# janelia-flyem/flypylib

Hardware: AMD Instinct MI355X
Metric: inference Mvoxels/sec, vgg_like (rf 18, 22^3 coarse -> 88^3 per reference tile), synthetic EM uint8 volume (higher is better)
Workload: dtype f16s; 1 GPU; the 520^3 volume of BASELINE.json's metric (configs[0]'s substack size) per GPU: vgg_like inference, 520x520x520 synthetic uint8 volume, reference tile lattice 102^3 (pitch 88), u8 in / f32 out resident in HBM; tile_in=102, executor=vgg_split_f16, parallelism=z-slab tile sharding x1, no collective, device=AMD Radeon Graphics (gfx950:sramecc+:xnack-)

## Files before the change

flypylib_amd/csrc/vgg_split.hip:

```cpp
#define FPL_F16 1
#include <algorithm>
#include <cmath>

#include "fast_paths.h"
#include "mfma_util.h"
#include "pack_weights.h"
#include <type_traits>
#include "vgg_split_lds.h"
#include "vgg_tiles.h"

namespace {

constexpr int CH = 48;
constexpr int CHP = 24, NPASS = CH / CHP;
constexpr int LO_OFF = CHP * 2;
constexpr int PASS_BYTES = 2 * LO_OFF;
constexpr int VOX = NPASS * PASS_BYTES;
constexpr int KS = (27 * CHP + 31) / 32;
constexpr int KTAB = (KS + 4) / 4 * 4;
constexpr int KTAB_BYTES = 4 * KTAB * 4;
static_assert(CHP % 8 == 0, "a lane's 8 k-slots stay inside one tap");

__host__ __device__ constexpr int64_t chan_off(int ch, int64_t plane) { return (ch / CHP) * plane + (ch % CHP) * 2; }

__device__ __forceinline__ h16x8 pack_relu_split_x(const f32x4 &blk) {
  u32x4 v;
  Pair2 p;
  p = split_pk_relu(blk[0], blk[1]); v[0] = p.hi; v[2] = p.lo;
  p = split_pk_relu(blk[2], blk[3]); v[1] = p.hi; v[3] = p.lo;
  return __builtin_bit_cast(h16x8, v);
}
__device__ __forceinline__ h16x8 pack_relu_split_x(const f32x4 &blk, unsigned &ovf) {
  const h16x8 r = pack_relu_split_x(blk);
  const u32x4 v = __builtin_bit_cast(u32x4, r);
  ovf_note(ovf, pk_max_i16(v[0], v[1]));
  return r;
}

__device__ __forceinline__ f32x4 chain48(const h16x8 (&w)[4], const Frag2 &h01, h16x8 hx, f32x4 acc) {
  acc = mfma16(w[1], h01.hi, acc);
  acc = mfma16(w[0], h01.lo, acc);
  acc = mfma16(w[2], hx, acc);
  acc = mfma16(w[3], hx, acc);
  return mfma16(w[0], h01.hi, acc);
}

__device__ __forceinline__ void store_split12(unsigned char *vox, int64_t plane, int g, const f32x4 (&v)[3],
                                              unsigned &ovf) {
  unsigned hi[6], lo[6];
#pragma unroll
  for (int b = 0; b < 3; ++b) {
    const Pair2 p0 = split_pk(v[b][0], v[b][1], ovf), p1 = split_pk(v[b][2], v[b][3], ovf);
    hi[2 * b] = p0.hi; hi[2 * b + 1] = p1.hi;
    lo[2 * b] = p0.lo; lo[2 * b + 1] = p1.lo;
  }
  unsigned char *d = vox + (g >> 1) * plane + 24 * (g & 1);
  *reinterpret_cast<u32x4_a8 *>(d) = u32x4_a8{hi[0], hi[1], hi[2], hi[3]};
  *reinterpret_cast<u32x2 *>(d + 16) = u32x2{hi[4], hi[5]};
  *reinterpret_cast<u32x4_a8 *>(d + LO_OFF) = u32x4_a8{lo[0], lo[1], lo[2], lo[3]};
  *reinterpret_cast<u32x2 *>(d + LO_OFF + 16) = u32x2{lo[4], lo[5]};
}

constexpr int S_PZ = 4, S_PY = 8, S_PX = 32;
constexpr int S_TZ = 2 * S_PZ + 2, S_TY = 2 * S_PY + 2, S_TX = 2 * S_PX + 2;
constexpr int S_TP = 80;
constexpr int S_TILE = S_TZ * S_TY * S_TP;
constexpr int S_WAVES = 8;
constexpr int S_ROWS = S_TZ * S_TY;
constexpr int S_WROWS = (S_ROWS + S_WAVES - 1) / S_WAVES;
constexpr int S_TASKS = S_PZ * S_PY * 2 / S_WAVES;
constexpr int S_RPT = 3;
static_assert(S_RPT * S_TASKS >= S_WROWS && S_WROWS <= 64, "stem fill schedule");
constexpr int S_SHTAB = 64 * 48;
constexpr int S_SH2 = 4 * 12;
constexpr int S_SMEM = 4 * S_TILE * 2 + 256 * 4 + S_SHTAB * 4 + 2 * S_SH2 * 4;

struct StemSArgs {
  const void *src;
  int64_t SZ, SY, SX;
  int64_t z_hi;
  float mean, sd;
  float c0;
  const float *shtab;
  int64_t p1z0;
  const h16x8 *w1, *w2;
  const float *shift1, *shift2;
  x8::Tensor p1;
  int nbx, nby, nbz;
  unsigned *flag;
  float xlim;
  unsigned char *dump;
};

__device__ __forceinline__ int stem_row_off(int row) {
  return ((row / 3) * S_TY + row % 3) * S_TP;
}

struct StemBlock {
  int px0, py0, pz0;
  int64_t gz0, gy0, gx0;
  unsigned xc;
  bool x_ok;
};

__device__ __forceinline__ StemBlock stem_block(const StemSArgs &a, int q, int lane) {
  StemBlock b;
  const int xb = q % a.nbx, t = q / a.nbx;
  const int yb = t % a.nby, zb = t / a.nby;
  b.px0 = xb * S_PX; b.py0 = yb * S_PY; b.pz0 = zb * S_PZ;
  b.gz0 = 2 * (a.p1z0 + b.pz0); b.gy0 = 2 * (int64_t)b.py0; b.gx0 = 2 * (int64_t)b.px0;
  const int64_t x = b.gx0 + lane;
  b.x_ok = x < a.SX;
  b.xc = (unsigned)(b.x_ok ? x : a.SX - 1);
  return b;
}

__device__ __forceinline__ int stem_row_of(int wrow0, int l) {
  const int r = wrow0 + (l < S_WROWS ? l : S_WROWS - 1);
  return r < S_ROWS ? r : S_ROWS - 1;
}

template <typename SRC>
__device__ __forceinline__ unsigned stem_row_tab(const StemSArgs &a, const StemBlock &b, int wrow0,
                                                 int lane, const SRC *&base) {
  const int row = stem_row_of(wrow0, lane);
  const int64_t z = b.gz0 + row / S_TY, y = b.gy0 + row % S_TY;
  const bool ok = z < a.z_hi && y < a.SY;
  const int64_t zc = z < a.z_hi ? z : a.z_hi - 1, yc = y < a.SY ? y : a.SY - 1;
  const int64_t zb = b.gz0 < a.z_hi ? b.gz0 : a.z_hi - 1, yb = b.gy0 < a.SY ? b.gy0 : a.SY - 1;
  base = (const SRC *)a.src + (zb * a.SY + yb) * a.SX;
  const unsigned rel = (unsigned)(((zc - zb) * a.SY + (yc - yb)) * a.SX);
  return rel | (ok ? 0x80000000u : 0u);
}

template <typename SRC>
struct StemRows {
  SRC v[S_RPT];
  bool ok[S_RPT];
};

template <typename SRC>
__device__ __forceinline__ void stem_load_rows(const SRC *base, unsigned tab, unsigned xc,
                                               int idx0, StemRows<SRC> &r) {
#pragma unroll
  for (int k = 0; k < S_RPT; ++k) {
    const int idx = idx0 + k < S_WROWS ? idx0 + k : S_WROWS - 1;
    const unsigned t = (unsigned)__builtin_amdgcn_readlane((int)tab, idx);
    r.ok[k] = (t >> 31) != 0u;
    r.v[k] = (base + (t & 0x7FFFFFFFu))[xc];
  }
}

template <typename SRC>
__device__ __forceinline__ unsigned stem_norm(const StemSArgs &a, const unsigned *lut, SRC v,
                                              bool ok, unsigned &xmax) {
  unsigned t;
  if (sizeof(SRC) == 1) {
    t = lut[(unsigned)v & 255u];
  } else {
    const float x = ((float)v - a.mean) / a.sd;
    const unsigned ax = __builtin_bit_cast(unsigned, x) & 0x7FFFFFFFu;
    xmax = ax > xmax ? ax : xmax;
    const h16_t h = (h16_t)x;
    t = (unsigned)h16_bits(x) | ((unsigned)h16_bits(x - (float)h) << 16);
  }
  return ok ? t : 0u;
}

struct StemBits { unsigned b[S_RPT]; };

template <typename SRC>
__device__ __forceinline__ void stem_convert_rows(const StemSArgs &a, const StemBlock &b,
                                                  const unsigned *lut, const StemRows<SRC> &r,
                                                  StemBits &o, unsigned &xmax) {
#pragma unroll
  for (int k = 0; k < S_RPT; ++k) o.b[k] = stem_norm<SRC>(a, lut, r.v[k], r.ok[k] && b.x_ok, xmax);
}

template <bool LO>
__device__ __forceinline__ void stem_write_rows(unsigned short *tile, int wrow0, int idx0, int lane,
                                                const StemBits &o) {
#pragma unroll
  for (int k = 0; k < S_RPT; ++k) {
    const int e = stem_row_of(wrow0, idx0 + k) * S_TP + lane;
    tile[e] = (unsigned short)o.b[k];
    if (LO) tile[S_TILE + e] = (unsigned short)(o.b[k] >> 16);
  }
}

template <typename SRC>
struct StemEdge { SRC v[2]; bool ok[2]; };

template <typename SRC>
__device__ __forceinline__ void stem_load_edge(const StemSArgs &a, const StemBlock &b, int wrow0,
                                               int lane, StemEdge<SRC> &e) {
  const int row = stem_row_of(wrow0, lane);
  const int64_t z = b.gz0 + row / S_TY, y = b.gy0 + row % S_TY;
  const bool rok = z < a.z_hi && y < a.SY;
  const int64_t zc = z < a.z_hi ? z : a.z_hi - 1, yc = y < a.SY ? y : a.SY - 1;
  const SRC *rp = (const SRC *)a.src + (zc * a.SY + yc) * a.SX;
#pragma unroll
  for (int j = 0; j < 2; ++j) {
    const int64_t x = b.gx0 + 64 + j;
    e.ok[j] = rok && x < a.SX;
    e.v[j] = rp[x < a.SX ? x : a.SX - 1];
  }
}

template <typename SRC>
__device__ __forceinline__ void stem_store_edge(const StemSArgs &a, unsigned short *tile,
                                                const unsigned *lut, int wrow0, int lane,
                                                const StemEdge<SRC> &e, unsigned &xmax) {
  const int row = stem_row_of(wrow0, lane);
  const unsigned v0 = stem_norm<SRC>(a, lut, e.v[0], e.ok[0], xmax);
  const unsigned v1 = stem_norm<SRC>(a, lut, e.v[1], e.ok[1], xmax);
  *reinterpret_cast<unsigned *>(&tile[row * S_TP + 64]) = (v0 & 0xFFFFu) | (v1 << 16);
  if (sizeof(SRC) != 1)
    *reinterpret_cast<unsigned *>(&tile[S_TILE + row * S_TP + 64]) = (v0 >> 16) | (v1 & 0xFFFF0000u);
}

extern __shared__ __attribute__((aligned(16))) unsigned char smem[];

template <typename SRC>
__global__ __launch_bounds__(64 * S_WAVES, 2) void vggs_stem_pool(StemSArgs a) {
  unsigned short *tiles = reinterpret_cast<unsigned short *>(smem);
  unsigned *lut = reinterpret_cast<unsigned *>(smem + 4 * S_TILE * 2);
  const int tid = threadIdx.x, lane = tid & 63;
  const int wave = __builtin_amdgcn_readfirstlane(tid >> 6);
  const int c = lane & 15, g = lane >> 4;
  const int nblocks = a.nbx * a.nby * a.nbz;
  int q = blockIdx.x;
  if (q >= nblocks) return;
  constexpr bool INT = sizeof(SRC) == 1;
  if (INT && tid < 256) lut[tid] = (unsigned)h16_bits((float)tid - a.c0);
  const unsigned char *shtab = smem + 4 * S_TILE * 2 + 256 * 4;
  if (INT)
    for (int i = tid; i < S_SHTAB; i += 64 * S_WAVES)
      reinterpret_cast<float *>(smem + 4 * S_TILE * 2 + 256 * 4)[i] = a.shtab[i];

  int offP[2][3], offS[2][2];
#pragma unroll
  for (int e = 0; e < 2; ++e) {
#pragma unroll
    for (int i = 0; i < 3; ++i)
      offP[e][i] = 2 * (g < 3 ? stem_row_off(3 * g + i) + (e == 0 ? 0 : 2)
                              : stem_row_off(6 + i) + (e == 0 ? 2 : 0));
#pragma unroll
    for (int h = 0; h < 2; ++h)
      offS[e][h] = 2 * (stem_row_off(2 * (g < 3 ? g : 2) + h) + (e == 0 ? 2 : 1));
  }
  h16x8 w1[2][2][3], w2[4][3];
  float *sh2t = reinterpret_cast<float *>(smem + 4 * S_TILE * 2 + 256 * 4 + S_SHTAB * 4);
  if (tid < S_SH2) {
    const float v = a.shift2[x8::out_channel((tid % 12) / 4, tid / 12, tid % 4)];
    sh2t[tid] = v;
    sh2t[S_SH2 + tid] = -v;
  }
  const f32x4 *sh2g = reinterpret_cast<const f32x4 *>(sh2t + 12 * g);
  const f32x4 *sh2n = reinterpret_cast<const f32x4 *>(sh2t + S_SH2 + 12 * g);
  f32x4 sh1[3];
#pragma unroll
  for (int p = 0; p < 2; ++p)
#pragma unroll
    for (int s = 0; s < 2; ++s)
#pragma unroll
      for (int b = 0; b < 3; ++b) {
        w1[p][s][b] = a.w1[((p * 2 + s) * 3 + b) * 64 + lane];
        w2[2 * p + s][b] = a.w2[((2 * p + s) * 3 + b) * 64 + lane];
      }
#pragma unroll
  for (int b = 0; b < 3; ++b)
#pragma unroll
    for (int r = 0; r < 4; ++r) {
      sh1[b][r] = a.shift1[16 * b + 4 * g + r];
    }
  __syncthreads();

  unsigned ovf = 0u, xmax = 0u;
  const int wrow0 = wave * S_WROWS;
  StemBlock blk = stem_block(a, q, lane);
  {
    const SRC *base0;
    const unsigned tab0 = stem_row_tab<SRC>(a, blk, wrow0, lane, base0);
    for (int i0 = 0; i0 < S_WROWS; i0 += S_RPT) {
      StemRows<SRC> rr;
      StemBits hb;
      stem_load_rows<SRC>(base0, tab0, blk.xc, i0, rr);
      stem_convert_rows<SRC>(a, blk, lut, rr, hb, xmax);
      stem_write_rows<!INT>(tiles, wrow0, i0, lane, hb);
    }
    StemEdge<SRC> ee;
    stem_load_edge<SRC>(a, blk, wrow0, lane, ee);
    stem_store_edge<SRC>(a, tiles, lut, wrow0, lane, ee, xmax);
  }
  __syncthreads();

  const int G = (int)gridDim.x;
  auto clampq = [&](int qq, int qlast) { return qq < nblocks ? qq : qlast; };
  StemRows<SRC> rr;
  StemEdge<SRC> ee;
  StemBits hb;
  {
    const StemBlock n0 = stem_block(a, clampq(q + G, q), lane);
    const SRC *bn;
    const unsigned tn = stem_row_tab<SRC>(a, n0, wrow0, lane, bn);
    stem_load_rows<SRC>(bn, tn, n0.xc, 0, rr);
    stem_load_edge<SRC>(a, n0, wrow0, lane, ee);
    stem_convert_rows<SRC>(a, n0, lut, rr, hb, xmax);
    stem_load_rows<SRC>(bn, tn, n0.xc, S_RPT, rr);
    const f32x4 z3[3] = {{0.f, 0.f, 0.f, 0.f}, {0.f, 0.f, 0.f, 0.f}, {0.f, 0.f, 0.f, 0.f}};
    __builtin_amdgcn_sched_barrier(0);
    x8::store12_sel(a.p1, 0, g, z3, ovf, false, a.dump);
  }
  struct Gin {
    unsigned p[INT ? 1 : 2][3], s0[INT ? 1 : 2], s1[INT ? 1 : 2];
  };
  struct Geo { int base, xrel, yrel, zrel, pzl, pyl, xh; };
  int cur = 0;
  for (;;) {
    const int qn = q + G;
    const bool has_next = qn < nblocks;
    const StemBlock nxt = stem_block(a, has_next ? qn : q, lane);
    const StemBlock nx2 = stem_block(a, clampq(qn + G, has_next ? qn : q), lane);
    const SRC *base_n, *base_2;
    const unsigned tab_n = stem_row_tab<SRC>(a, nxt, wrow0, lane, base_n);
    const unsigned tab_2 = stem_row_tab<SRC>(a, nx2, wrow0, lane, base_2);
    const unsigned char *tb = reinterpret_cast<const unsigned char *>(tiles + cur * 2 * S_TILE);
    unsigned short *tnext = tiles + (cur ^ 1) * 2 * S_TILE;
    auto geo = [&](int ti) {
      Geo t;
      const int task = wave + S_WAVES * ti;
      const int row = task >> 1;
      t.xh = task & 1; t.pzl = row / S_PY; t.pyl = row % S_PY;
      t.base = 2 * (((2 * t.pzl) * S_TY + 2 * t.pyl) * S_TP + 2 * (16 * t.xh + c));
      t.xrel = (int)(blk.gx0 + 2 * (16 * t.xh + c) + 3 - a.SX);
      t.yrel = (int)(blk.gy0 + 2 * t.pyl + 3 - a.SY);
      t.zrel = (int)(blk.gz0 + 2 * t.pzl + 3 - a.z_hi);
      return t;
    };
    const bool interior = INT && blk.gx0 + 2 * S_PX + 2 <= a.SX && blk.gy0 + 2 * S_PY + 2 <= a.SY &&
                          blk.gz0 + 2 * S_PZ + 2 <= a.z_hi;
    auto block_pass = [&](auto edge_t) {
      constexpr bool EDGE = decltype(edge_t)::value;
      f32x4 kin[3];
      if (INT && !EDGE) {
#pragma unroll
        for (int b = 0; b < 3; ++b) kin[b] = *reinterpret_cast<const f32x4 *>(shtab + (4 * g) * 4 + 64 * b);
      }
      auto gather = [&](const Geo &t, int sub, Gin &o) {
        const int sp = sub >> 1, e = sub & 1;
        const int so = 2 * ((((sp >> 1) & 1) * S_TY + (sp & 1)) * S_TP);
#pragma unroll
        for (int part = 0; part < (INT ? 1 : 2); ++part) {
          const unsigned char *tp = tb + part * (S_TILE * 2) + t.base + so;
#pragma unroll
          for (int i = 0; i < 3; ++i) o.p[part][i] = *reinterpret_cast<const unsigned *>(tp + offP[e][i]);
          o.s0[part] = *reinterpret_cast<const unsigned short *>(tp + offS[e][0]);
          o.s1[part] = *reinterpret_cast<const unsigned short *>(tp + offS[e][1]);
        }
      };
      auto gather_init = [&](const Geo &t, int sub, f32x4 (&o)[3]) {
        if (INT && EDGE) {
          const int sp = sub >> 1, e = sub & 1;
          const int pzy = 4 * min(max(t.zrel + (sp >> 1), 0), 3) + min(max(t.yrel + (sp & 1), 0), 3);
          const unsigned char *tp = shtab + ((4 * pzy + min(max(t.xrel + e, 0), 3)) * 48 + 4 * g) * 4;
#pragma unroll
          for (int b = 0; b < 3; ++b) o[b] = *reinterpret_cast<const f32x4 *>(tp + 64 * b);
        }
      };
      auto frag = [&](const Gin &gi, int part) {
        const u32x4 raw = {gi.p[part][0], gi.p[part][1], gi.p[part][2], gi.s0[part] | (gi.s1[part] << 16)};
        return __builtin_bit_cast(h16x8, raw);
      };
      constexpr int NC3 = INT ? 6 : 9;
      auto c3 = [&](int i, int e, const f32x4 (&gin)[3], h16x8 bh, h16x8 bl, f32x4 (&o)[3]) {
        const int b = i % 3, grp = i / 3;
        if (grp == 0) o[b] = mfma16(w1[1][e][b], bh, INT ? (EDGE ? gin[b] : kin[b]) : sh1[b]);
        else if (!INT && grp == 1) o[b] = mfma16(w1[0][e][b], bl, o[b]);
        else o[b] = mfma16(w1[0][e][b], bh, o[b]);
      };
      constexpr int NGB = INT ? 2 : 1, DEPTH = NGB + 1;
      Gin Gd[NGB];
      f32x4 gin[3];
      f32x4 a1n[3];
      f32x4 a2[2][3];
      f32x4 poolf[3];
#pragma unroll
      for (int b = 0; b < 3; ++b) poolf[b] = sh2n[b];
#pragma unroll
      for (int e = 0; e < 2; ++e)
#pragma unroll
        for (int b = 0; b < 3; ++b) a2[e][b] = f32x4{0.f, 0.f, 0.f, 0.f};
      {
        const Geo t0 = geo(0);
        gather(t0, 0, Gd[0]);
        gather_init(t0, 0, gin);
        const h16x8 bh = frag(Gd[0], 0), bl = INT ? bh : frag(Gd[0], INT ? 0 : 1);
#pragma unroll
        for (int i = 0; i < NC3; ++i) c3(i, 0, gin, bh, bl, a1n);
        gather_init(t0, 1, gin);
#pragma unroll
        for (int q = 1; q < DEPTH; ++q) gather(t0, q, Gd[q % NGB]);
      }
#pragma unroll 1
      for (int ti = 0; ti < S_TASKS; ++ti) {
        const bool conv2 = ti + 1 >= S_TASKS, load2 = ti + 2 >= S_TASKS;
        const SRC *lbase = load2 ? base_2 : base_n;
        const unsigned ltab = load2 ? tab_2 : tab_n, lxc = load2 ? nx2.xc : nxt.xc;
        const int lidx = S_RPT * ((ti + 2) & (S_TASKS - 1));
        const Geo tg = geo(ti), tn = geo((ti + 1) & (S_TASKS - 1)), tp = geo((ti + S_TASKS - 1) & (S_TASKS - 1));
#pragma unroll
        for (int sub = 0; sub < 8; ++sub) {
          const int sp = sub >> 1, e = sub & 1, en = e ^ 1;
          f32x4 a1[3];
#pragma unroll
          for (int b = 0; b < 3; ++b) a1[b] = a1n[b];
          const Gin &G = Gd[(sub + 1) % NGB];
          const h16x8 bh = frag(G, 0), bl = INT ? bh : frag(G, INT ? 0 : 1);
          float r[12];
          unsigned hi[6], lo[6];
          auto A = [&](int p) {
            r[2 * p] = relu_f32(a1[p >> 1][2 * (p & 1)]);
            r[2 * p + 1] = relu_f32(a1[p >> 1][2 * (p & 1) + 1]);
            hi[p] = cvt_pk_h16(r[2 * p], r[2 * p + 1]);
          };
          auto B = [&](int p) {
            lo[p] = split_lo_pk(r[2 * p], hi[p], r[2 * p + 1]);
          };
          auto PL = [&](int k) {
#pragma unroll
            for (int j = 2 * k; j < 2 * k + 2; ++j)
              poolf[j >> 2][j & 3] = __builtin_fmaxf(__builtin_fmaxf(poolf[j >> 2][j & 3], a2[0][j >> 2][j & 3]),
                                                     a2[1][j >> 2][j & 3]);
          };
          auto c1 = [&](int i) {
            const int b = i % 3, grp = i / 3;
            const u32x4 h0h = {hi[0], hi[1], hi[2], hi[3]}, h0l = {lo[0], lo[1], lo[2], lo[3]};
            const u32x4 hxv = {hi[4], hi[5], lo[4], lo[5]};
            if (grp == 0) a2[e][b] = mfma16(w2[1][b], __builtin_bit_cast(h16x8, h0h), f32x4{0.f, 0.f, 0.f, 0.f});
            if (grp == 1) a2[e][b] = mfma16(w2[0][b], __builtin_bit_cast(h16x8, h0h), a2[e][b]);
            if (grp == 2) a2[e][b] = mfma16(w2[0][b], __builtin_bit_cast(h16x8, h0l), a2[e][b]);
            if (grp == 3) a2[e][b] = mfma16(w2[2][b], __builtin_bit_cast(h16x8, hxv), a2[e][b]);
            if (grp == 4) a2[e][b] = mfma16(w2[3][b], __builtin_bit_cast(h16x8, hxv), a2[e][b]);
          };
#pragma unroll
          for (int s = 0; s < 15; ++s) {
            if (s < 6) c3(s, en, gin, bh, bl, a1n);
            else c1(s - 6);
            if (s < 6 && e == 0) PL(s);
            if (s < 4) A(s);
            else if (s < 8) B(s - 4);
            else if (s < 10) A(s - 4);
            else if (s < 12) B(s - 6);
            __builtin_amdgcn_sched_barrier(0);
          }
          if (sub + DEPTH < 8) gather(tg, sub + DEPTH, Gd[(sub + DEPTH) % NGB]);
          else gather(tn, sub + DEPTH - 8, Gd[(sub + DEPTH) % NGB]);
          if (sub + 2 < 8) gather_init(tg, sub + 2, gin);
          else gather_init(tn, sub + 2 - 8, gin);
#pragma unroll
          for (int i = 6; i < NC3; ++i) c3(i, en, gin, bh, bl, a1n);
#pragma unroll
          for (int i = 9; i < 15; ++i) c1(i);
          if (sub == 0) {
            const int pz = blk.pz0 + tp.pzl, py = blk.py0 + tp.pyl, px = blk.px0 + 16 * tp.xh + c;
            f32x4 pv[3];
#pragma unroll
            for (int b = 0; b < 3; ++b) pv[b] = poolf[b] + sh2g[b];
            x8::store12_sel(a.p1, a.p1.vox(pz, py, px), g, pv, ovf,
                            ti > 0 && pz < a.p1.Z && py < a.p1.Y && px < a.p1.X, a.dump);
#pragma unroll
            for (int b = 0; b < 3; ++b) poolf[b] = sh2n[b];
          }
          if (sub == 3) stem_write_rows<!INT>(tnext, wrow0, S_RPT * ti, lane, hb);
          if (sub == 5) {
#pragma unroll
            for (int k = 0; k < S_RPT; ++k) {
              unsigned t = sizeof(SRC) == 1 ? (unsigned)rr.v[k] : __builtin_bit_cast(unsigned, (float)rr.v[k]);
              asm volatile("" : "+v"(t));
              rr.v[k] = sizeof(SRC) == 1 ? (SRC)t : (SRC)__builtin_bit_cast(float, t);
            }
            stem_convert_rows<SRC>(a, conv2 ? nx2 : nxt, lut, rr, hb, xmax);
          }
          if (sub == 7) stem_load_rows<SRC>(lbase, ltab, lxc, lidx, rr);
          __builtin_amdgcn_sched_barrier(0);
        }
      }
      {
        const Geo t7 = geo(S_TASKS - 1);
#pragma unroll
        for (int b = 0; b < 3; ++b)
#pragma unroll
          for (int r = 0; r < 4; ++r)
            poolf[b][r] = __builtin_fmaxf(__builtin_fmaxf(poolf[b][r], a2[0][b][r]), a2[1][b][r]);
        const int pz = blk.pz0 + t7.pzl, py = blk.py0 + t7.pyl, px = blk.px0 + 16 * t7.xh + c;
        f32x4 pv[3];
#pragma unroll
        for (int b = 0; b < 3; ++b) pv[b] = poolf[b] + sh2g[b];
        x8::store12_sel(a.p1, a.p1.vox(pz, py, px), g, pv, ovf,
                        pz < a.p1.Z && py < a.p1.Y && px < a.p1.X, a.dump);
      }
    };
    if (interior) block_pass(std::false_type{});
    else block_pass(std::true_type{});
    if (!has_next) break;
    stem_store_edge<SRC>(a, tnext, lut, wrow0, lane, ee, xmax);
    stem_load_edge<SRC>(a, nx2, wrow0, lane, ee);
    __syncthreads();
    q = qn;
    blk = nxt;
    cur ^= 1;
  }
  ovf_commit(ovf, a.flag, FPL_RANGE_STEM);
  if (!INT && xmax > __builtin_bit_cast(unsigned, a.xlim)) atomicOr(a.flag, FPL_RANGE_INPUT);
}

template <int TY, int TX>
__device__ __forceinline__ unsigned kslot_entry(int idx) {
  const int g = idx / KTAB;
  int s = idx % KTAB;
  s = s < KS ? s : KS - 1;
  const int f0 = 32 * s + 8 * g;
  const int tap = f0 / CHP, ch0 = f0 % CHP;
  if (tap >= 27) return 0u;
  return (unsigned)((((tap / 9) * TY + (tap / 3) % 3) * TX + tap % 3) * PASS_BYTES + ch0 * 2);
}

constexpr int WQ = 2;

template <typename Fill, typename SubOff>
__device__ __forceinline__ void conv3s_kloop_f(Fill fill, unsigned char *tile,
                                               const unsigned *kofftab, const unsigned char *wglobal,
                                               unsigned vbase, SubOff sub_off, f32x4 (&acc)[4][3],
                                               int tid) {
  const int lane = tid & 63, wave = tid >> 6, g = lane >> 4;
  const unsigned *ktab = kofftab + g * KTAB;
#pragma unroll 1
  for (int pass = 0; pass < NPASS; ++pass) {
    if (pass) __syncthreads();
    fill(pass);
    const unsigned char *wl = wglobal + (size_t)pass * KS * 6 * 1024 + lane * 16;
    h16x8 wq[WQ][6];
#pragma unroll
    for (int d = 0; d < WQ; ++d)
#pragma unroll
      for (int f = 0; f < 6; ++f)
        wq[d][f] = *reinterpret_cast<const h16x8 *>(wl + (size_t)(d * 6 + f) * 1024);
    __syncthreads();
    u32x4 kv = *reinterpret_cast<const u32x4 *>(ktab);
    Frag2 bcur[4], bnxt[4];
#pragma unroll
    for (int sub = 0; sub < 4; ++sub) {
      const unsigned char *p = tile + vbase + kv[0] + sub_off(sub);
      bcur[sub].hi = *reinterpret_cast<const h16x8 *>(p);
      bcur[sub].lo = *reinterpret_cast<const h16x8 *>(p + LO_OFF);
    }
#pragma unroll
    for (int s = 0; s < KS; ++s) {
      if ((s + 1) % 4 == 0) kv = *reinterpret_cast<const u32x4 *>(ktab + s + 1);
      const unsigned koff = kv[(s + 1) % 4];
#pragma unroll
      for (int sub = 0; sub < 4; ++sub) {
        const unsigned char *p = tile + vbase + koff + sub_off(sub);
        bnxt[sub].hi = *reinterpret_cast<const h16x8 *>(p);
        bnxt[sub].lo = *reinterpret_cast<const h16x8 *>(p + LO_OFF);
      }
      __builtin_amdgcn_s_setprio(1);
#pragma unroll
      for (int sub = 0; sub < 4; ++sub)
#pragma unroll
        for (int b = 0; b < 3; ++b) acc[sub][b] = mfma16(wq[s % WQ][3 + b], bcur[sub].hi, acc[sub][b]);
#pragma unroll
      for (int sub = 0; sub < 4; ++sub)
#pragma unroll
        for (int b = 0; b < 3; ++b) acc[sub][b] = mfma16(wq[s % WQ][b], bcur[sub].lo, acc[sub][b]);
#pragma unroll
      for (int sub = 0; sub < 4; ++sub)
#pragma unroll
        for (int b = 0; b < 3; ++b) acc[sub][b] = mfma16(wq[s % WQ][b], bcur[sub].hi, acc[sub][b]);
      __builtin_amdgcn_s_setprio(0);
      if (s + WQ < KS) {
#pragma unroll
        for (int f = 0; f < 6; ++f)
          wq[s % WQ][f] = *reinterpret_cast<const h16x8 *>(wl + (size_t)((s + WQ) * 6 + f) * 1024);
      }
#pragma unroll
      for (int sub = 0; sub < 4; ++sub) bcur[sub] = bnxt[sub];
    }
  }
}

template <int TZ, int TY, int TX, typename SubOff>
__device__ __forceinline__ void conv3s_kloop(const unsigned char *act, int AZ, int AY, int AX,
                                             int z0, int y0, int x0, unsigned char *tile,
                                             const unsigned *kofftab, const unsigned char *wglobal,
                                             unsigned vbase, SubOff sub_off, f32x4 (&acc)[4][3],
                                             int tid) {
  const int lane = tid & 63, wave = tid >> 6;
  auto fill = [&](int pass) {
    stage_tile<TZ, TY, TX, PASS_BYTES, PASS_BYTES>(act + (int64_t)pass * AZ * AY * AX * PASS_BYTES, AZ, AY, AX,
                                                   z0, y0, x0, tile, wave, lane);
  };
  conv3s_kloop_f(fill, tile, kofftab, wglobal, vbase, sub_off, acc, tid);
}

constexpr int M_TZ = 6, M_TY = 6, M_TX = 18;
constexpr int M_TILE_BYTES = ((M_TZ * M_TY * M_TX * PASS_BYTES + 1023) / 1024) * 1024;
constexpr int M_SMEM = M_TILE_BYTES + KTAB_BYTES;
static_assert(2 * M_SMEM <= 160 * 1024, "two workgroups must fit one CU");

struct MidXArgs {
  x8::Tensor p1;
  const unsigned char *w3;
  const h16x8 *w4;
  const float *shift3, *shift4;
  x8::Tensor p2;
  x8::Walk walk;
  unsigned *flag;
};

__global__ __launch_bounds__(64 * x8::WAVES, 2) void vggs_mid_pool(MidXArgs a) {
  unsigned *ktab = reinterpret_cast<unsigned *>(smem + 2 * x8::BUF);
  const int tid = threadIdx.x, lane = tid & 63;
  const int wave = __builtin_amdgcn_readfirstlane(tid >> 6);
  const int c = lane & 15, g = lane >> 4;
  x8::ktab_init(ktab, tid);
  const x8::TileDma td = x8::tile_dma_init(wave, lane, a.p1.Y, a.p1.XP, (unsigned)a.p1.part_bytes());
  const int S = (int)gridDim.x >> 3, nbricks = a.walk.bricks();
  const int group = (int)blockIdx.x & 7, slot = (int)blockIdx.x >> 3;
  x8::Cursor cur;
  if (!x8::cursor_first(a.walk, nbricks, group, slot, S, cur)) return;
  const int64_t part = a.p1.part_bytes();
  auto origin = [&](const x8::Cursor &q) {
    return a.p1.p + a.p1.vox(8 * q.bz, 4 * q.by, 16 * q.bx) * 16;
  };
  const int pzl = wave >> 1, pyl = wave & 1;
  const unsigned vb = (unsigned)(((2 * pzl) * x8::ZS + (2 * pyl) * x8::TX + c) * 16);
  auto sub_off = [](int sub) -> unsigned { return (unsigned)((((sub >> 1) & 1) * x8::ZS + (sub & 1) * x8::TX) * 16); };
  unsigned ovf_all = 0u;
  x8::prime(smem, td, origin(cur), part, a.w3, wave, lane);
  for (;;) {
    x8::Cursor nxt = cur;
    const bool has_next = x8::cursor_next(a.walk, slot, S, nxt);
    int zero = 0;
    asm volatile("" : "+s"(zero));
    f32x4 acc[4][3];
#pragma unroll
    for (int b = 0; b < 3; ++b) {
      const f32x4 sh = *reinterpret_cast<const f32x4 *>(a.shift3 + zero + 16 * b + 4 * g);
#pragma unroll
      for (int sub = 0; sub < 4; ++sub) acc[sub][b] = sh;
    }
    x8::conv_block(smem, ktab + 8 * g, td, origin(cur), origin(has_next ? nxt : cur), part, a.w3, vb,
                   sub_off, wave, lane, acc);
    asm volatile("" : "+s"(zero));
    const h16x8 *w4p = a.w4 + zero;
    f32x4 sh4[3];
// ... 668 lines not shown
  }
  for (uint16_t h : st->w1_int_host)
    if ((h & 0x7C00u) == 0x7C00u)
      return fpl_fail_range_call(ctx, "a first-layer weight divided by std %g exceeds the IEEE-half range; use "
                                 "precision f32 (or 'auto') for this normalisation", (double)sd);
  if (!(stem_input_limit(A, op, scale.data(), st->shift1_int_host.data(), 64) >= std::max(c0, 255.0 - c0)))
    return fpl_fail_range_call(ctx, "the first layer's outputs may exceed the IEEE-half range at mean %g, std %g; "
                               "use precision f32 (or 'auto')", (double)mean, (double)sd);
  const size_t wb = st->w1_int_host.size() * sizeof(uint16_t);
  if (!st->w1_int) FPL_HIP(ctx, hipMalloc((void **)&st->w1_int, wb));
  if (!st->shift1_int) FPL_HIP(ctx, hipMalloc((void **)&st->shift1_int, S_SHTAB * sizeof(float)));
  FPL_HIP(ctx, hipMemcpyAsync(st->w1_int, st->w1_int_host.data(), wb, hipMemcpyHostToDevice, ctx->stream));
  FPL_HIP(ctx, hipMemcpyAsync(st->shift1_int, st->shift1_int_host.data(), S_SHTAB * sizeof(float),
                              hipMemcpyHostToDevice, ctx->stream));
  st->int_c0 = (float)c0;
  st->int_mean = mean; st->int_sd = sd;
  st->int_valid = true;
  return 0;
}

}

bool fpl_split_path_available(const fpl_program *prog, int precision, const int32_t offset[3],
                              const int32_t out_sz[3]) {
  const int variant = fpl_vgg_variant(prog);
  if (precision != FPL_PREC_F16S || variant == 0) return false;
  for (int a = 0; a < 3; ++a)
    if (offset[a] != (variant == 1 ? 7 : 10) || out_sz[a] % 4 != 0) return false;
  return true;
}

namespace {

int split2_infer(fpl_ctx *ctx, SplitState *st, const void *src, int src_dtype, float mean, float sd,
                 const int64_t dims[3], const std::vector<int32_t> origins[3],
                 const int32_t out_sz[3], int32_t zb, int32_t ze, float *dst) {
  hipStream_t stream = ctx->stream;
  constexpr int OFF = 10;
  const int64_t SZ = dims[0], SY = dims[1], SX = dims[2];
  const int64_t VZ = SZ - 2 * OFF, VY = SY - 2 * OFF, VX = SX - 2 * OFF;
  if (VZ <= 0 || VY <= 0 || VX <= 0 || zb >= ze) return 0;
  const int64_t fz_lo = (int64_t)origins[0][zb] - OFF;
  const int64_t fz_hi = std::min<int64_t>((int64_t)origins[0][ze - 1] - OFF + out_sz[0], VZ);
  const int64_t cz_lo = fz_lo / 4, cz_hi = ceil_div64(fz_hi, 4);
  const int CY = (int)ceil_div64(VY, 4), CX = (int)ceil_div64(VX, 4);
  const int QY = CY + 2, QX = CX + 2, T3Y = 2 * QY + 2, T3X = 2 * QX + 2, HY = T3Y + 2, HX = T3X + 2;
  const int64_t h_row = (int64_t)HY * HX * VOX, t_row = (int64_t)T3Y * T3X * VOX;
  const char *budget_env = getenv("FPL_VGG_SCRATCH_MB");
  const int64_t budget = budget_env ? (int64_t)atoll(budget_env) << 20 : (int64_t)64 << 30;
  int64_t cz_chunk = std::max<int64_t>(4, (budget / (h_row + t_row) - 8) / 2);
  cz_chunk = std::min<int64_t>(cz_chunk, cz_hi - cz_lo);
  cz_chunk = (cz_chunk + 3) / 4 * 4;
  FPL_REQUIRE(ctx, (int64_t)HY * HX * PASS_BYTES * 8 < ((int64_t)1 << 32),
              "vgg_like2 split path: a %lld x %lld plane is too large for the tile loader's 32-bit "
              "offsets", (long long)SY, (long long)SX);
  DevTemp tmp(ctx);
  unsigned *flag;
  FPL_TRY(fpl_range_flag(ctx, &flag));
  void *h1v, *l3v, *qv;
  FPL_TRY(tmp.alloc((size_t)(2 * cz_chunk + 8) * h_row, &h1v));
  FPL_TRY(tmp.alloc((size_t)(2 * cz_chunk + 6) * t_row, &l3v));
  FPL_TRY(tmp.alloc((size_t)(cz_chunk + 2) * QY * QX * VOX, &qv));
  const unsigned char *F = st->frags;
  const float *S = st->shifts;
  for (int64_t c0 = cz_lo; c0 < cz_hi; c0 += cz_chunk) {
    const int CZ = (int)std::min<int64_t>(cz_chunk, cz_hi - c0);
    const int QZ = CZ + 2, T3Z = 2 * QZ + 2, HZ = T3Z + 2;
    {
      V2SArgs a = {};
      a.src = src; a.SZ = SZ; a.SY = SY; a.SX = SX; a.mean = mean; a.sd = sd;
      a.gz0 = 4 * c0;
      a.wstem = (const h16x8 *)(F + st->off_w[0]); a.shstem = S + st->off_s[0];
      if (src_dtype == FPL_U8) {
        a.wstem = (const h16x8 *)st->w1_int; a.shtab = st->shift1_int; a.c0 = st->int_c0;
      }
      a.w = F + st->off_w[1]; a.shift = S + st->off_s[1];
      a.out = (unsigned char *)h1v; a.OZ = HZ; a.OY = HY; a.OX = HX;
      a.flag = flag; a.xlim = st->xlim;
      a.bg = BlockGrid{(int)ceil_div64(HX, 8), (int)ceil_div64(HY, 2), (int)ceil_div64(HZ, 2)};
      TimedLaunch tl(ctx, "vggs2_stem_conv3_pool");
      if (src_dtype == FPL_U8)
        vggs2_conv3<true, true, uint8_t><<<brick_grid_size(a.bg), 256, V2_SMEM, stream>>>(a);
      else
        vggs2_conv3<true, true, float><<<brick_grid_size(a.bg), 256, V2_SMEM, stream>>>(a);
    }
    {
      V2SArgs a = {};
      a.in = (const unsigned char *)h1v; a.IZ = HZ; a.IY = HY; a.IX = HX;
      a.w = F + st->off_w[2]; a.shift = S + st->off_s[2];
      a.out = (unsigned char *)l3v; a.OZ = T3Z; a.OY = T3Y; a.OX = T3X;
      a.flag = flag;
      a.bg = BlockGrid{(int)ceil_div64(T3X, 16), (int)ceil_div64(T3Y, 4), (int)ceil_div64(T3Z, 4)};
      TimedLaunch tl(ctx, "vggs2_conv3");
      vggs2_conv3<false, false, uint8_t><<<brick_grid_size(a.bg), 256, V2_SMEM, stream>>>(a);
    }
    {
      V2SArgs a = {};
      a.in = (const unsigned char *)l3v; a.IZ = T3Z; a.IY = T3Y; a.IX = T3X;
      a.w = F + st->off_w[3]; a.shift = S + st->off_s[3];
      a.out = (unsigned char *)qv; a.OZ = QZ; a.OY = QY; a.OX = QX;
      a.flag = flag;
      a.bg = BlockGrid{(int)ceil_div64(QX, 8), (int)ceil_div64(QY, 2), (int)ceil_div64(QZ, 2)};
      TimedLaunch tl(ctx, "vggs2_conv3_pool");
      vggs2_conv3<false, true, uint8_t><<<brick_grid_size(a.bg), 256, V2_SMEM, stream>>>(a);
    }
    {
      TailSArgs a;
      a.p2 = (const unsigned char *)qv; a.P2Z = QZ; a.P2Y = QY; a.P2X = QX;
      a.w5 = F + st->off_w[4]; a.shift5 = S + st->off_s[4];
      a.CZ = CZ; a.CY = CY; a.CX = CX;
      a.w6 = F + st->off_w[5]; a.w7 = F + st->off_w[6]; a.w8 = F + st->off_w[7];
      a.shift6 = S + st->off_s[5]; a.shift7 = S + st->off_s[6]; a.bias8 = st->bias8;
      a.dst = dst; a.DY = SY; a.DX = SX; a.gz0 = c0;
      a.VZ = std::min<int64_t>(fz_hi, VZ); a.VY = VY; a.VX = VX; a.off = OFF;
      a.flag = flag;
      a.bg = BlockGrid{(int)ceil_div64(CX, 16), (int)ceil_div64(CY, 4), (int)ceil_div64(CZ, 4)};
      TimedLaunch tl(ctx, "vggs_c5_tail");
      vggs_c5_tail_p24<<<brick_grid_size(a.bg), 256, M_SMEM, stream>>>(a);
    }
    FPL_HIP(ctx, hipGetLastError());
  }
  return 0;
}

}

static int x8_pitch(int X) { return X; }

int fpl_split_infer_volume(fpl_ctx *ctx, fpl_program *prog, const void *src, int src_dtype,
                           float mean, float sd, const int64_t dims[3],
                           const std::vector<int32_t> origins[3], const int32_t out_sz[3],
                           int32_t zb, int32_t ze, float *dst) {
  SplitState *st;
  FPL_TRY(split_prepare(ctx, prog, &st));
  if (src_dtype == FPL_U8) FPL_TRY(split_prepare_int(ctx, prog, st, mean, sd));
  if (fpl_vgg_variant(prog) == 2)
    return split2_infer(ctx, st, src, src_dtype, mean, sd, dims, origins, out_sz, zb, ze, dst);
  hipStream_t stream = ctx->stream;
  const int64_t SZ = dims[0], SY = dims[1], SX = dims[2];
  const int64_t VZ = SZ - 14, VY = SY - 14, VX = SX - 14;
  if (VZ <= 0 || VY <= 0 || VX <= 0 || zb >= ze) return 0;
  const int64_t fz_lo = (int64_t)origins[0][zb] - 7;
  const int64_t fz_hi = std::min<int64_t>((int64_t)origins[0][ze - 1] - 7 + out_sz[0], VZ);
  const int64_t cz_lo = fz_lo / 4, cz_hi = ceil_div64(fz_hi, 4);
  const int CY = (int)ceil_div64(VY, 4), CX = (int)ceil_div64(VX, 4);
  const int P2Y = CY + 2, P2X = CX + 2, P1Y = 2 * P2Y + 2, P1X = 2 * P2X + 2;
  const int P1XP = x8_pitch(P1X), P2XP = x8_pitch(P2X);
  const int64_t p1_row_bytes = (int64_t)P1Y * P1XP * VOX;
  const char *budget_env = getenv("FPL_VGG_SCRATCH_MB");
  const int64_t budget = budget_env ? (int64_t)atoll(budget_env) << 20 : (int64_t)64 << 30;
  int64_t cz_chunk = std::max<int64_t>(4, (budget / p1_row_bytes - 6) / 2);
  cz_chunk = std::min<int64_t>(cz_chunk, cz_hi - cz_lo);
  cz_chunk = (cz_chunk + 3) / 4 * 4;
  FPL_REQUIRE(ctx, (int64_t)S_TZ * SY * SX < ((int64_t)1 << 31),
              "vgg split path: a %lld x %lld plane is too large for the stem's 31-bit row "
              "offsets", (long long)SY, (long long)SX);
  {
    const int64_t max_rows = (((int64_t)1 << 32) / 16 / ((int64_t)P1Y * P1XP) - (x8::TZ + 2));
    FPL_REQUIRE(ctx, max_rows >= 14,
                "vgg split path: a %lld x %lld plane is too large for the tile loader's 32-bit "
                "offsets", (long long)SY, (long long)SX);
    cz_chunk = std::min<int64_t>(cz_chunk, std::max<int64_t>(4, ((max_rows - 6) / 2) / 4 * 4));
  }
  DevTemp tmp(ctx);
  unsigned *flag;
  FPL_TRY(fpl_range_flag(ctx, &flag));
  x8::Tensor p1 = {nullptr, (int)(2 * cz_chunk + 6), P1Y, P1X, P1XP}, p2 = {nullptr, (int)(cz_chunk + 2), P2Y, P2X, P2XP};
  void *p1v, *p2v;
  FPL_TRY(tmp.alloc((size_t)(p1.bytes() + p1.slack_bytes()), &p1v));
  FPL_TRY(tmp.alloc((size_t)(p2.bytes() + p2.slack_bytes()), &p2v));
  void *dumpv;
  FPL_TRY(tmp.alloc(256, &dumpv));
  const unsigned pgrid = (unsigned)std::max(8, ctx->n_cu / 8 * 8);
  const unsigned char *F = st->frags;
  const float *S = st->shifts;
  for (int64_t c0 = cz_lo; c0 < cz_hi; c0 += cz_chunk) {
    const int CZ = (int)std::min<int64_t>(cz_chunk, cz_hi - c0);
    const int P2Z = CZ + 2, P1Z = 2 * P2Z + 2;
    p1 = x8::Tensor{(unsigned char *)p1v, P1Z, P1Y, P1X, P1XP};
    p2 = x8::Tensor{(unsigned char *)p2v, P2Z, P2Y, P2X, P2XP};
    FPL_HIP(ctx, hipMemsetAsync(p1.p + p1.bytes(), 0, (size_t)p1.slack_bytes(), stream));
    FPL_HIP(ctx, hipMemsetAsync(p2.p + p2.bytes(), 0, (size_t)p2.slack_bytes(), stream));
    {
      StemSArgs a;
      a.src = src; a.SZ = SZ; a.SY = SY; a.SX = SX; a.mean = mean; a.sd = sd;
      a.p1z0 = 2 * c0;
      a.z_hi = std::min<int64_t>(SZ, 4 * (c0 + CZ) + 14);
      a.w1 = (const h16x8 *)(F + st->off_w[0]);
      a.w2 = (const h16x8 *)(F + st->off_w[1]);
      a.shift1 = S + st->off_s[0]; a.shift2 = S + st->off_s[1];
      a.c0 = 0.f; a.shtab = nullptr;
      if (src_dtype == FPL_U8) {
        a.w1 = (const h16x8 *)st->w1_int; a.shtab = st->shift1_int;
        a.c0 = st->int_c0;
      }
      a.p1 = p1;
      a.flag = flag; a.xlim = st->xlim; a.dump = (unsigned char *)dumpv;
      a.nbx = (int)ceil_div64(P1X, S_PX); a.nby = (int)ceil_div64(P1Y, S_PY);
      a.nbz = (int)ceil_div64(P1Z, S_PZ);
      const unsigned grid = (unsigned)std::min<int64_t>((int64_t)a.nbx * a.nby * a.nbz,
                                                        (int64_t)ctx->n_cu);
      TimedLaunch tl(ctx, "vggs_stem_pool");
      if (src_dtype == FPL_U8)
        vggs_stem_pool<uint8_t><<<grid, 64 * S_WAVES, S_SMEM, stream>>>(a);
      else
        vggs_stem_pool<float><<<grid, 64 * S_WAVES, S_SMEM, stream>>>(a);
    }
    {
      MidXArgs a;
      a.p1 = p1;
      a.w3 = F + st->off_w[2];
      a.w4 = (const h16x8 *)(F + st->off_w[3]);
      a.shift3 = S + st->off_s[2]; a.shift4 = S + st->off_s[3];
      a.p2 = p2;
      a.flag = flag;
      a.walk = x8::Walk{(int)ceil_div64(P2X, 8), (int)ceil_div64(P2Y, 2), (int)ceil_div64(P2Z, 4)};
      TimedLaunch tl(ctx, "vggs_mid_pool");
      vggs_mid_pool<<<pgrid, 64 * x8::WAVES, x8::SMEM, stream>>>(a);
    }
    {
      TailXArgs a;
      a.p2 = p2;
      a.w5 = F + st->off_w[4]; a.shift5 = S + st->off_s[4];
      a.CZ = CZ; a.CY = CY; a.CX = CX;
      a.w6 = F + st->off_w[5]; a.w7 = F + st->off_w[6]; a.w8 = F + st->off_w[7];
      a.shift6 = S + st->off_s[5]; a.shift7 = S + st->off_s[6]; a.bias8 = st->bias8;
      a.dst = dst; a.DY = SY; a.DX = SX; a.gz0 = c0;
      a.VZ = std::min<int64_t>(fz_hi, VZ); a.VY = VY; a.VX = VX; a.off = 7;
      a.flag = flag;
      a.walk = x8::Walk{(int)ceil_div64(CX, 16), (int)ceil_div64(CY, 4), (int)ceil_div64(CZ, 8)};
      TimedLaunch tl(ctx, "vggs_c5_tail");
      vggs_c5_tail<<<pgrid, 64 * x8::WAVES, x8::SMEM, stream>>>(a);
    }
    FPL_HIP(ctx, hipGetLastError());
  }
  return 0;
}
```

Before: 15200 Mvoxels/s.

## Trim stem work on partial edge blocks by remapping lanes to live voxels

For stem blocks that extend past the p1 tensor bounds, a trimmed task schedule packs lanes onto only the live output voxels. It picks an x-tile width of 4, 8 or 16 based on the remaining extent, so fewer task iterations run. Because the pipelined prefetch of the next block's rows would otherwise be cut short, a fallback loads and converts the skipped rows after the pass. The path is gated by FPL_VGG_EDGE_BLOCKS and on by default. It adds a third template instantiation (code size, register pressure) and changes the order of the software pipeline on edge blocks.

```diff
diff --git a/flypylib_amd/csrc/vgg_split.hip b/flypylib_amd/csrc/vgg_split.hip
--- a/flypylib_amd/csrc/vgg_split.hip
+++ b/flypylib_amd/csrc/vgg_split.hip
@@ -87,6 +87,7 @@
   const float *shift1, *shift2;
   x8::Tensor p1;
   int nbx, nby, nbz;
+  int trim;
   unsigned *flag;
   float xlim;
   unsigned char *dump;
@@ -217,6 +218,29 @@
   *reinterpret_cast<unsigned *>(&tile[row * S_TP + 64]) = (v0 & 0xFFFFu) | (v1 << 16);
   if (sizeof(SRC) != 1)
     *reinterpret_cast<unsigned *>(&tile[S_TILE + row * S_TP + 64]) = (v0 >> 16) | (v1 & 0xFFFF0000u);
+}
+
+struct StemTrim {
+  int pxs;
+  int ntx, nty;
+  int nt;
+  int mag;
+};
+
+__device__ __forceinline__ StemTrim stem_trim(const StemSArgs &a, const StemBlock &b) {
+  StemTrim t;
+  const int lx = min(S_PX, a.p1.X - b.px0), ly = min(S_PY, a.p1.Y - b.py0), lz = min(S_PZ, a.p1.Z - b.pz0);
+  t.pxs = lx > 8 ? 4 : lx > 4 ? 3 : 2;
+  const int pyh = 16 >> t.pxs;
+  t.ntx = (lx + (1 << t.pxs) - 1) >> t.pxs;
+  t.nty = (ly + pyh - 1) / pyh;
+  t.nt = lz * t.nty * t.ntx;
+  t.mag = (1024 + t.nty - 1) / t.nty;
+  return t;
+}
+
+__device__ __forceinline__ bool stem_full(const StemSArgs &a, const StemBlock &b) {
+  return b.px0 + S_PX <= a.p1.X && b.py0 + S_PY <= a.p1.Y && b.pz0 + S_PZ <= a.p1.Z;
 }
 
 extern __shared__ __attribute__((aligned(16))) unsigned char smem[];
@@ -315,7 +339,7 @@
   struct Gin {
     unsigned p[INT ? 1 : 2][3], s0[INT ? 1 : 2], s1[INT ? 1 : 2];
   };
-  struct Geo { int base, xrel, yrel, zrel, pzl, pyl, xh; };
+  struct Geo { int base, xrel, yrel, zrel, pzl, pyl, pxl; bool live; };
   int cur = 0;
   for (;;) {
     const int qn = q + G;
@@ -331,17 +355,40 @@
       Geo t;
       const int task = wave + S_WAVES * ti;
       const int row = task >> 1;
-      t.xh = task & 1; t.pzl = row / S_PY; t.pyl = row % S_PY;
-      t.base = 2 * (((2 * t.pzl) * S_TY + 2 * t.pyl) * S_TP + 2 * (16 * t.xh + c));
-      t.xrel = (int)(blk.gx0 + 2 * (16 * t.xh + c) + 3 - a.SX);
+      const int xh = task & 1;
+      t.pzl = row / S_PY; t.pyl = row % S_PY; t.pxl = 16 * xh + c; t.live = true;
+      t.base = 2 * (((2 * t.pzl) * S_TY + 2 * t.pyl) * S_TP + 2 * (16 * xh + c));
+      t.xrel = (int)(blk.gx0 + 2 * (16 * xh + c) + 3 - a.SX);
+      t.yrel = (int)(blk.gy0 + 2 * t.pyl + 3 - a.SY);
+      t.zrel = (int)(blk.gz0 + 2 * t.pzl + 3 - a.z_hi);
+      return t;
+    };
+    const StemTrim trm = stem_trim(a, blk);
+    auto geo_trim = [&](int ti) {
+      Geo t;
+      int task = wave + S_WAVES * ti;
+      t.live = task < trm.nt;
+      task = t.live ? task : trm.nt - 1;
+      const int r = task >> (trm.ntx - 1), tx = task & (trm.ntx - 1);
+      const int tz = (r * trm.mag) >> 10, ty = r - tz * trm.nty;
+      t.pzl = tz;
+      t.pyl = (ty << (4 - trm.pxs)) + (c >> trm.pxs);
+      t.pxl = (tx << trm.pxs) + (c & ((1 << trm.pxs) - 1));
+      t.base = 2 * (((2 * t.pzl) * S_TY + 2 * t.pyl) * S_TP + 2 * t.pxl);
+      t.xrel = (int)(blk.gx0 + 2 * t.pxl + 3 - a.SX);
       t.yrel = (int)(blk.gy0 + 2 * t.pyl + 3 - a.SY);
       t.zrel = (int)(blk.gz0 + 2 * t.pzl + 3 - a.z_hi);
       return t;
     };
     const bool interior = INT && blk.gx0 + 2 * S_PX + 2 <= a.SX && blk.gy0 + 2 * S_PY + 2 <= a.SY &&
                           blk.gz0 + 2 * S_PZ + 2 <= a.z_hi;
-    auto block_pass = [&](auto edge_t) {
-      constexpr bool EDGE = decltype(edge_t)::value;
+    auto block_pass = [&](auto edge_t, auto trim_t) {
+      constexpr bool EDGE = decltype(edge_t)::value, TRIM = decltype(trim_t)::value;
+      auto gg = [&](int ti) {
+        if constexpr (TRIM) return geo_trim(ti);
+        else return geo(ti);
+      };
+      const int ntask = TRIM ? max(1, (trm.nt - wave + S_WAVES - 1) / S_WAVES) : S_TASKS;
       f32x4 kin[3];
       if (INT && !EDGE) {
 #pragma unroll
@@ -392,7 +439,7 @@
 #pragma unroll
         for (int b = 0; b < 3; ++b) a2[e][b] = f32x4{0.f, 0.f, 0.f, 0.f};
       {
-        const Geo t0 = geo(0);
+        const Geo t0 = gg(0);
         gather(t0, 0, Gd[0]);
         gather_init(t0, 0, gin);
         const h16x8 bh = frag(Gd[0], 0), bl = INT ? bh : frag(Gd[0], INT ? 0 : 1);
@@ -403,12 +450,12 @@
         for (int q = 1; q < DEPTH; ++q) gather(t0, q, Gd[q % NGB]);
       }
 #pragma unroll 1
-      for (int ti = 0; ti < S_TASKS; ++ti) {
+      for (int ti = 0; ti < ntask; ++ti) {
         const bool conv2 = ti + 1 >= S_TASKS, load2 = ti + 2 >= S_TASKS;
         const SRC *lbase = load2 ? base_2 : base_n;
         const unsigned ltab = load2 ? tab_2 : tab_n, lxc = load2 ? nx2.xc : nxt.xc;
         const int lidx = S_RPT * ((ti + 2) & (S_TASKS - 1));
-        const Geo tg = geo(ti), tn = geo((ti + 1) & (S_TASKS - 1)), tp = geo((ti + S_TASKS - 1) & (S_TASKS - 1));
+        const Geo tg = gg(ti), tn = gg((ti + 1) & (S_TASKS - 1)), tp = gg((ti + S_TASKS - 1) & (S_TASKS - 1));
 #pragma unroll
         for (int sub = 0; sub < 8; ++sub) {
           const int sp = sub >> 1, e = sub & 1, en = e ^ 1;
@@ -463,12 +510,12 @@
 #pragma unroll
           for (int i = 9; i < 15; ++i) c1(i);
           if (sub == 0) {
-            const int pz = blk.pz0 + tp.pzl, py = blk.py0 + tp.pyl, px = blk.px0 + 16 * tp.xh + c;
+            const int pz = blk.pz0 + tp.pzl, py = blk.py0 + tp.pyl, px = blk.px0 + tp.pxl;
             f32x4 pv[3];
 #pragma unroll
             for (int b = 0; b < 3; ++b) pv[b] = poolf[b] + sh2g[b];
             x8::store12_sel(a.p1, a.p1.vox(pz, py, px), g, pv, ovf,
-                            ti > 0 && pz < a.p1.Z && py < a.p1.Y && px < a.p1.X, a.dump);
+                            ti > 0 && tp.live && pz < a.p1.Z && py < a.p1.Y && px < a.p1.X, a.dump);
 #pragma unroll
             for (int b = 0; b < 3; ++b) poolf[b] = sh2n[b];
           }
@@ -487,22 +534,46 @@
         }
       }
       {
-        const Geo t7 = geo(S_TASKS - 1);
+        const Geo t7 = gg(ntask - 1);
 #pragma unroll
         for (int b = 0; b < 3; ++b)
 #pragma unroll
           for (int r = 0; r < 4; ++r)
             poolf[b][r] = __builtin_fmaxf(__builtin_fmaxf(poolf[b][r], a2[0][b][r]), a2[1][b][r]);
-        const int pz = blk.pz0 + t7.pzl, py = blk.py0 + t7.pyl, px = blk.px0 + 16 * t7.xh + c;
+        const int pz = blk.pz0 + t7.pzl, py = blk.py0 + t7.pyl, px = blk.px0 + t7.pxl;
         f32x4 pv[3];
 #pragma unroll
         for (int b = 0; b < 3; ++b) pv[b] = poolf[b] + sh2g[b];
         x8::store12_sel(a.p1, a.p1.vox(pz, py, px), g, pv, ovf,
-                        pz < a.p1.Z && py < a.p1.Y && px < a.p1.X, a.dump);
+                        t7.live && pz < a.p1.Z && py < a.p1.Y && px < a.p1.X, a.dump);
+      }
+      if (TRIM && ntask < S_TASKS) {
+        stem_write_rows<!INT>(tnext, wrow0, S_RPT * ntask, lane, hb);
+        constexpr int FB = INT ? S_TASKS - 1 : 4;
+        StemRows<SRC> f8;
+        stem_load_rows<SRC>(base_2, tab_2, nx2.xc, 0, f8);
+        stem_load_rows<SRC>(base_2, tab_2, nx2.xc, S_RPT, rr);
+#pragma unroll
+        for (int j0 = 0; j0 < S_TASKS - 1; j0 += FB) {
+          StemRows<SRC> fr[FB];
+#pragma unroll
+          for (int j = 0; j < FB; ++j)
+            if (j0 + j < S_TASKS - 1 && ntask + 1 + j0 + j < S_TASKS)
+              stem_load_rows<SRC>(base_n, tab_n, nxt.xc, S_RPT * (ntask + 1 + j0 + j), fr[j]);
+#pragma unroll
+          for (int j = 0; j < FB; ++j)
+            if (j0 + j < S_TASKS - 1 && ntask + 1 + j0 + j < S_TASKS) {
+              StemBits fb;
+              stem_convert_rows<SRC>(a, nxt, lut, fr[j], fb, xmax);
+              stem_write_rows<!INT>(tnext, wrow0, S_RPT * (ntask + 1 + j0 + j), lane, fb);
+            }
+        }
+        stem_convert_rows<SRC>(a, nx2, lut, f8, hb, xmax);
       }
     };
-    if (interior) block_pass(std::false_type{});
-    else block_pass(std::true_type{});
+    if (a.trim && !stem_full(a, blk)) block_pass(std::true_type{}, std::true_type{});
+    else if (interior) block_pass(std::false_type{}, std::false_type{});
+    else block_pass(std::true_type{}, std::false_type{});
     if (!has_next) break;
     stem_store_edge<SRC>(a, tnext, lut, wrow0, lane, ee, xmax);
     stem_load_edge<SRC>(a, nx2, wrow0, lane, ee);
@@ -1477,6 +1548,8 @@
   int64_t cz_chunk = std::max<int64_t>(4, (budget / p1_row_bytes - 6) / 2);
   cz_chunk = std::min<int64_t>(cz_chunk, cz_hi - cz_lo);
   cz_chunk = (cz_chunk + 3) / 4 * 4;
+  const char *edge_env = getenv("FPL_VGG_EDGE_BLOCKS");
+  const int edge_blocks = edge_env ? atoi(edge_env) != 0 : 1;
   FPL_REQUIRE(ctx, (int64_t)S_TZ * SY * SX < ((int64_t)1 << 31),
               "vgg split path: a %lld x %lld plane is too large for the stem's 31-bit row "
               "offsets", (long long)SY, (long long)SX);
@@ -1523,6 +1596,7 @@
       a.flag = flag; a.xlim = st->xlim; a.dump = (unsigned char *)dumpv;
       a.nbx = (int)ceil_div64(P1X, S_PX); a.nby = (int)ceil_div64(P1Y, S_PY);
       a.nbz = (int)ceil_div64(P1Z, S_PZ);
+      a.trim = edge_blocks;
       const unsigned grid = (unsigned)std::min<int64_t>((int64_t)a.nbx * a.nby * a.nbz,
                                                         (int64_t)ctx->n_cu);
       TimedLaunch tl(ctx, "vggs_stem_pool");
```

Result: faster. 15650 Mvoxels/s (median of 6 runs) (+3.0%).
